# riffusion/riffusion-hobby

Hardware: NVIDIA H100
Metric: clips/sec (higher is better)
Workload: dtype f16

## Files before the change

### riffusion-hobby_b200/csrc/rf_gemm.cu

```cuda
#include <cuda.h>
#include <cuda_fp16.h>
#include <cuda_runtime.h>

#include <algorithm>
#include <cstdio>
#include <cstdlib>
#include <mutex>
#include <string>
#include <vector>

#include "rf_common.h"
#include "rf_tc.cuh"

namespace {

constexpr int BM = 128;
constexpr int BK = 64;
constexpr int A_TILE_BYTES = BM * BK * 2;
constexpr int GEMM_THREADS = 256 + 32;
constexpr int STAGE_PAD = 4;

__host__ __device__ constexpr int stage_bytes(int BN) { return BM * (BN + STAGE_PAD) * 4; }

struct TcParams {
    int M, N, K;
    int batch1, batch2;
    int num_kb;
    int tiles_m, tiles_n;
    int a_m1, a_m2, b_m1, b_m2;
    int conv;
    int taps;
    int kc1, kc2;
    int stride, pad;
    int tap_w;
    int off_x, off_y;
    int osx, osy, oox, ooy;
    int HoF, WoF;
    int Ho, Wo, Bn;
    int bw, bh, bb;
    int tiles_x, tiles_y;
    __half* out;
    long ldo, so1, so2;
    const __half* bias;
    int bias_mode;
    const __half* bias2;
    int bias2_pitch;
    const __half* residual;
    long ldr, sr1, sr2;
    float alpha;
    int act;
    float* out_f32;
    int splits, kb_per_split;
    float* ws;
    long ws_split_stride;
};

__device__ __forceinline__ float apply_act(float v, int act) {
    if (act == 1) return __fdividef(v, 1.f + __expf(-v));
    if (act == 3) return __fdividef(v, 1.f + __expf(-1.702f * v));
    return v;
}

__device__ __forceinline__ float gelu_erf_fast(float g) {
    const float t = fminf(fabsf(g) * 0.70710678118654752f, 4.0f);
    float q = -2.1777638e-05f;
    q = fmaf(q, t, 0.0005068331f);
    q = fmaf(q, t, -0.005339398f);
    q = fmaf(q, t, 0.034231447f);
    q = fmaf(q, t, -0.15289085f);
    q = fmaf(q, t, -0.91675895f);
    q = fmaf(q, t, -1.6281544f);
    q = fmaf(q, t, -0.9999938f);
    float h;
    asm("ex2.approx.ftz.f32 %0, %1;" : "=f"(h) : "f"(q));
    return g * (g < 0.f ? (t < 4.0f ? h : 0.f) : 1.f - h);
}

__device__ __forceinline__ void named_bar_sync(int id, int n) { asm volatile("bar.sync %0, %1;" ::"r"(id), "r"(n) : "memory"); }

constexpr int BRES_KB = 5;
template <int BN, int STAGES, bool BRES = false>
__global__ void __launch_bounds__(GEMM_THREADS, 1)
k_tc_gemm(const __grid_constant__ CUtensorMap mapA0, const __grid_constant__ CUtensorMap mapA1,
          const __grid_constant__ CUtensorMap mapB, const TcParams p) {
    extern __shared__ __align__(1024) uint8_t smem[];
    rf_pdl_trigger();
    constexpr int B_TILE_BYTES = BN * BK * 2;
    constexpr int PITCH = BN + STAGE_PAD;
    uint8_t* sA = smem;
    uint8_t* sB = smem + STAGES * A_TILE_BYTES;
    float* stg = reinterpret_cast<float*>(sB + (BRES ? BRES_KB : STAGES) * B_TILE_BYTES);
    uint64_t* full = reinterpret_cast<uint64_t*>(reinterpret_cast<uint8_t*>(stg) + stage_bytes(BN));
    uint64_t* empty = full + STAGES;
    uint64_t* b_full = empty + STAGES;

    const int warp = threadIdx.x >> 5, lane = threadIdx.x & 31;
    const int tiles_mn = p.tiles_n * p.tiles_m;
    const int n_tiles = tiles_mn * p.batch1 * p.batch2 * p.splits;
    const int nb_fixed = BRES ? static_cast<int>(blockIdx.x) % p.tiles_n : 0;
    const int unit0 = BRES ? static_cast<int>(blockIdx.x) / p.tiles_n : blockIdx.x;
    const int unit_step = BRES ? static_cast<int>(gridDim.x) / p.tiles_n : gridDim.x;
    const int n_units = BRES ? p.tiles_m : n_tiles;

    if (threadIdx.x == 0) {
        for (int i = 0; i < STAGES; ++i) {
            tc::mbar_init(&full[i], 1);
            tc::mbar_init(&empty[i], 256);
        }
        tc::mbar_init(b_full, 1);
        tc::fence_barrier_init();
    }
    if (warp == 8 && lane == 0) {
        tc::tma_prefetch_desc(&mapA0);
        tc::tma_prefetch_desc(&mapB);
    }
    __syncthreads();
    rf_pdl_wait();

    if (warp == 8) {
        if (lane != 0) return;
        int it = 0;
        if constexpr (BRES) {
            tc::mbar_expect_tx(b_full, p.num_kb * B_TILE_BYTES);
            for (int kb = 0; kb < p.num_kb; ++kb)
                tc::tma_load_4d(&mapB, b_full, sB + kb * B_TILE_BYTES, kb * BK, nb_fixed * BN, 0, 0);
        }
        for (int unit = unit0; unit < n_units; unit += unit_step) {
            const int tile = BRES ? unit * p.tiles_n + nb_fixed : unit / p.splits, sp = BRES ? 0 : unit - (unit / p.splits) * p.splits;
            const int kb0 = sp * p.kb_per_split, kb1 = min(p.num_kb, kb0 + p.kb_per_split);
            const int z = tile / tiles_mn, mn = tile - z * tiles_mn;
            const int m_blk = mn / p.tiles_n, n_blk = mn - m_blk * p.tiles_n;
            const int b1 = z % p.batch1, b2 = z / p.batch1;
            int tx = 0, ty = 0, tb = 0;
            if (p.conv) {
                tx = m_blk % p.tiles_x;
                ty = (m_blk / p.tiles_x) % p.tiles_y;
                tb = m_blk / (p.tiles_x * p.tiles_y);
            }
            for (int kb = kb0; kb < kb1; ++kb, ++it) {
                const int stage = it % STAGES;
                const uint32_t phase = (it / STAGES) & 1;
                tc::mbar_wait(&empty[stage], phase ^ 1);
                tc::mbar_expect_tx(&full[stage], A_TILE_BYTES + (BRES ? 0 : B_TILE_BYTES));
                void* dstA = sA + stage * A_TILE_BYTES;
                void* dstB = sB + stage * B_TILE_BYTES;
                if (!p.conv) {
                    tc::tma_load_4d(&mapA0, &full[stage], dstA, kb * BK, m_blk * BM, b1 * p.a_m1, b2 * p.a_m2);
                    if (!BRES) tc::tma_load_4d(&mapB, &full[stage], dstB, kb * BK, n_blk * BN, b1 * p.b_m1, b2 * p.b_m2);
                } else {
                    const int kct = p.kc1 + p.kc2;
                    const int tap = kb / kct, kc = kb - tap * kct;
                    const int dy = tap / p.tap_w, dx = tap - dy * p.tap_w;
                    const int x0 = tx * p.bw * p.stride + dx - p.pad + p.off_x;
                    const int y0 = ty * p.bh * p.stride + dy - p.pad + p.off_y;
                    if (kc < p.kc1)
                        tc::tma_load_4d(&mapA0, &full[stage], dstA, kc * BK, x0, y0, tb * p.bb);
                    else
                        tc::tma_load_4d(&mapA1, &full[stage], dstA, (kc - p.kc1) * BK, x0, y0, tb * p.bb);
                    if (!BRES) tc::tma_load_4d(&mapB, &full[stage], dstB, kb * BK, n_blk * BN, 0, 0);
                }
            }
        }
        return;
    }

    const int wg = warp >> 2;
    const int frag_row = wg * 64 + (warp & 3) * 16 + (lane >> 2), frag_col = 2 * (lane & 3);
    const int row = threadIdx.x & 127;
    const int half_id = threadIdx.x >> 7;
    auto ld64 = [](const __half* src, uint4* q4) {
        const uint4* s4 = reinterpret_cast<const uint4*>(src);
#pragma unroll
        for (int j = 0; j < 4; ++j) q4[j] = s4[j];
    };
    if constexpr (BRES) tc::mbar_wait(b_full, 0);
    int it = 0;
    for (int unit = unit0; unit < n_units; unit += unit_step) {
        const int tile = BRES ? unit * p.tiles_n + nb_fixed : unit / p.splits, sp = BRES ? 0 : unit - (unit / p.splits) * p.splits;
        const int kb0 = sp * p.kb_per_split, kb1 = min(p.num_kb, kb0 + p.kb_per_split);
        float acc[BN / 2];
#pragma unroll
        for (int i = 0; i < BN / 2; ++i) acc[i] = 0.f;
        int prev = -1;
        for (int kb = kb0; kb < kb1; ++kb, ++it) {
            const int stage = it % STAGES;
            tc::mbar_wait(&full[stage], (it / STAGES) & 1);
            const uint32_t a_base = tc::smem_u32(sA + stage * A_TILE_BYTES) + wg * (64 * 128);
            const uint32_t b_base = tc::smem_u32(sB + (BRES ? kb : stage) * B_TILE_BYTES);
            tc::wgmma_fence();
#pragma unroll
            for (int k = 0; k < BK / 16; ++k)
                tc::wgmma_ss<BN>(acc, tc::make_desc_sw128(a_base + k * 32), tc::make_desc_sw128(b_base + k * 32), 1u);
            tc::wgmma_commit();
            tc::wgmma_wait<1>();
            tc::reg_fence<BN / 2>(acc);
            if (prev >= 0) tc::mbar_arrive(&empty[prev]);
            prev = stage;
        }
        tc::wgmma_wait<0>();
        tc::reg_fence<BN / 2>(acc);
        if (prev >= 0) tc::mbar_arrive(&empty[prev]);

        named_bar_sync(1, 256);
#pragma unroll
        for (int i = 0; i < BN / 8; ++i) {
            const int c = 8 * i + frag_col;
            *reinterpret_cast<float2*>(stg + frag_row * PITCH + c) = make_float2(acc[4 * i], acc[4 * i + 1]);
            *reinterpret_cast<float2*>(stg + (frag_row + 8) * PITCH + c) = make_float2(acc[4 * i + 2], acc[4 * i + 3]);
        }
        named_bar_sync(1, 256);

        const int z = tile / tiles_mn, mn = tile - z * tiles_mn;
        const int m_blk = mn / p.tiles_n, n_blk = mn - m_blk * p.tiles_n;
        const int b1 = z % p.batch1, b2 = z / p.batch1;
        bool row_ok;
        long out_off, res_off;
        int img = 0;
        if (!p.conv) {
            const int m = m_blk * BM + row;
            row_ok = m < p.M;
            out_off = static_cast<long>(b2) * p.so2 + static_cast<long>(b1) * p.so1 + static_cast<long>(m) * p.ldo;
            res_off = static_cast<long>(b2) * p.sr2 + static_cast<long>(b1) * p.sr1 + static_cast<long>(m) * p.ldr;
        } else {
            const int tx = m_blk % p.tiles_x, ty = (m_blk / p.tiles_x) % p.tiles_y, tb = m_blk / (p.tiles_x * p.tiles_y);
            const int xi = row % p.bw, yi = (row / p.bw) % p.bh, bi = row / (p.bw * p.bh);
            const int x = tx * p.bw + xi, y = ty * p.bh + yi;
            img = tb * p.bb + bi;
            row_ok = (x < p.Wo) && (y < p.Ho) && (img < p.Bn);
            const long pix = (static_cast<long>(img) * p.HoF + (y * p.osy + p.ooy)) * p.WoF + (x * p.osx + p.oox);
            out_off = pix * p.ldo;
            res_off = pix * p.ldr;
        }
        const int m_glob = m_blk * BM + row;
        const float bias_row = (p.bias_mode == 2 && row_ok) ? __half2float(p.bias[m_glob]) : 0.f;
#pragma unroll 1
        for (int c0 = half_id * 32; c0 < BN; c0 += 64) {
            const int n0 = n_blk * BN + c0;
            if (!row_ok || n0 >= p.N) continue;
            float f[32];
#pragma unroll
            for (int i = 0; i < 8; ++i) {
                const float4 t = *reinterpret_cast<const float4*>(stg + row * PITCH + c0 + 4 * i);
                f[4 * i] = t.x; f[4 * i + 1] = t.y; f[4 * i + 2] = t.z; f[4 * i + 3] = t.w;
            }
            if (p.splits > 1) {
                float* wp = p.ws + sp * p.ws_split_stride + (out_off / p.ldo) * p.N + n0;
                if (n0 + 32 <= p.N && (p.N & 3) == 0) {
#pragma unroll
                    for (int i = 0; i < 8; ++i)
                        reinterpret_cast<float4*>(wp)[i] = make_float4(f[4 * i], f[4 * i + 1], f[4 * i + 2], f[4 * i + 3]);
                } else {
                    for (int i = 0; i < 32; ++i)
                        if (n0 + i < p.N) wp[i] = f[i];
                }
                continue;
            }
#pragma unroll
            for (int i = 0; i < 32; ++i) f[i] = f[i] * p.alpha + bias_row;
            const bool full_run = n0 + 32 <= p.N;
            if (p.bias_mode == 1) {
                if (full_run && ((reinterpret_cast<uintptr_t>(p.bias + n0) & 15) == 0)) {
                    uint4 q4[4];
                    ld64(p.bias + n0, q4);
#pragma unroll
                    for (int j = 0; j < 4; ++j) {
                        const uint4 bv = q4[j];
                        const __half2* bh = reinterpret_cast<const __half2*>(&bv);
#pragma unroll
                        for (int e = 0; e < 4; ++e) {
                            const float2 t = __half22float2(bh[e]);
                            f[8 * j + 2 * e] += t.x;
                            f[8 * j + 2 * e + 1] += t.y;
                        }
                    }
                } else {
                    for (int i = 0; i < 32; ++i)
                        if (n0 + i < p.N) f[i] += __half2float(p.bias[n0 + i]);
                }
            }
            if (p.bias2) {
                const __half* b2p = p.bias2 + static_cast<long>(img) * p.bias2_pitch + n0;
                if (full_run && ((reinterpret_cast<uintptr_t>(b2p) & 15) == 0)) {
                    uint4 q4[4];
                    ld64(b2p, q4);
#pragma unroll
                    for (int j = 0; j < 4; ++j) {
                        const uint4 bv = q4[j];
                        const __half2* bh = reinterpret_cast<const __half2*>(&bv);
#pragma unroll
                        for (int e = 0; e < 4; ++e) {
                            const float2 t = __half22float2(bh[e]);
                            f[8 * j + 2 * e] += t.x;
                            f[8 * j + 2 * e + 1] += t.y;
                        }
                    }
                } else {
                    for (int i = 0; i < 32; ++i)
                        if (n0 + i < p.N) f[i] += __half2float(b2p[i]);
                }
            }
            if (p.act == 2) {
                __half* dst = p.out + out_off + (n0 >> 1);
                uint32_t pk[8];
#pragma unroll
                for (int j = 0; j < 8; ++j) {
                    const float g0 = f[16 + 2 * j], g1 = f[17 + 2 * j];
                    const float y0 = f[2 * j] * gelu_erf_fast(g0);
                    const float y1 = f[2 * j + 1] * gelu_erf_fast(g1);
                    const __half2 h = __floats2half2_rn(y0, y1);
                    pk[j] = *reinterpret_cast<const uint32_t*>(&h);
                }
                reinterpret_cast<uint4*>(dst)[0] = make_uint4(pk[0], pk[1], pk[2], pk[3]);
                reinterpret_cast<uint4*>(dst)[1] = make_uint4(pk[4], pk[5], pk[6], pk[7]);
                continue;
            }
            if (p.act) {
#pragma unroll
                for (int i = 0; i < 32; ++i) f[i] = apply_act(f[i], p.act);
            }
            if (p.residual) {
                const __half* rp = p.residual + res_off + n0;
                if (full_run && ((reinterpret_cast<uintptr_t>(rp) & 15) == 0)) {
                    uint4 q4[4];
                    ld64(rp, q4);
#pragma unroll
                    for (int j = 0; j < 4; ++j) {
                        const uint4 rv = q4[j];
                        const __half2* rh = reinterpret_cast<const __half2*>(&rv);
#pragma unroll
                        for (int e = 0; e < 4; ++e) {
                            const float2 t = __half22float2(rh[e]);
                            f[8 * j + 2 * e] += t.x;
                            f[8 * j + 2 * e + 1] += t.y;
                        }
                    }
                } else {
                    for (int i = 0; i < 32; ++i)
                        if (n0 + i < p.N) f[i] += __half2float(rp[i]);
                }
            }
            if (p.out_f32) {
                for (int i = 0; i < 32; ++i)
                    if (n0 + i < p.N) p.out_f32[out_off + n0 + i] = f[i];
            } else if (full_run && ((reinterpret_cast<uintptr_t>(p.out + out_off + n0) & 15) == 0)) {
                uint4* dst = reinterpret_cast<uint4*>(p.out + out_off + n0);
#pragma unroll
                for (int i = 0; i < 4; ++i) {
                    __half2 h0 = __floats2half2_rn(f[8 * i + 0], f[8 * i + 1]);
                    __half2 h1 = __floats2half2_rn(f[8 * i + 2], f[8 * i + 3]);
                    __half2 h2 = __floats2half2_rn(f[8 * i + 4], f[8 * i + 5]);
                    __half2 h3 = __floats2half2_rn(f[8 * i + 6], f[8 * i + 7]);
                    dst[i] = make_uint4(*reinterpret_cast<uint32_t*>(&h0), *reinterpret_cast<uint32_t*>(&h1),
                                        *reinterpret_cast<uint32_t*>(&h2), *reinterpret_cast<uint32_t*>(&h3));
                }
            } else {
                for (int i = 0; i < 32; ++i)
                    if (n0 + i < p.N) p.out[out_off + n0 + i] = __float2half_rn(f[i]);
            }
        }
    }
}

struct TcProfile {
    bool on = false;
    std::vector<cudaEvent_t> ev;
    double flops = 0.0;
    long launches = 0;
    struct Rec { int conv, M, N, K, batch, splits, bn; };
    std::vector<Rec> recs;
};

TcProfile g_prof;
std::mutex g_prof_mu;

template <int BN, int STAGES, bool BRES = false>
int launch(const CUtensorMap& a0, const CUtensorMap& a1, const CUtensorMap& b, const TcParams& p, dim3 grid,
           cudaStream_t st) {
    constexpr size_t smem = static_cast<size_t>(STAGES) * A_TILE_BYTES +
                            static_cast<size_t>(BRES ? BRES_KB : STAGES) * (BN * BK * 2) + stage_bytes(BN) + 1024;
    static_assert(smem <= 232448, "shared memory budget (227 KB per block)");
    const int num_sms = rf_num_sms();
    const int n_tiles = static_cast<int>(grid.x * grid.y * grid.z);
    if (BRES) {
        grid = dim3(static_cast<unsigned>((num_sms / p.tiles_n) * p.tiles_n));
    } else {
        grid = dim3(static_cast<unsigned>(n_tiles < num_sms ? n_tiles : num_sms));
    }
    static rf_dev_once once;
    const cudaError_t aerr = rf_set_smem_once(once, k_tc_gemm<BN, STAGES, BRES>, int(smem));
    if (aerr != cudaSuccess) return rf_fail(RF_ERR_CUDA, std::string("cudaFuncSetAttribute: ") + cudaGetErrorString(aerr));
    cudaEvent_t e0 = nullptr, e1 = nullptr;
    const bool prof = g_prof.on;
    if (prof) {
        RF_CUDA_TRY(cudaEventCreate(&e0));
        RF_CUDA_TRY(cudaEventCreate(&e1));
        RF_CUDA_TRY(cudaEventRecord(e0, st));
    }
    RF_LAUNCH_PDL("k_tc_gemm", (k_tc_gemm<BN, STAGES, BRES>), grid, dim3(GEMM_THREADS), smem, st, n_tiles <= 2 * num_sms,
                  a0, a1, b, p);
    if (prof) {
        RF_CUDA_TRY(cudaEventRecord(e1, st));
        std::lock_guard<std::mutex> lk(g_prof_mu);
        g_prof.ev.push_back(e0);
        g_prof.ev.push_back(e1);
        g_prof.launches += 1;
        const double m = p.conv ? static_cast<double>(p.Bn) * p.Ho * p.Wo : static_cast<double>(p.M) * p.batch1 * p.batch2;
        g_prof.flops += 2.0 * m * p.N * p.K;
        g_prof.recs.push_back({p.conv, p.conv ? p.Bn * p.Ho * p.Wo : p.M, p.N, p.K, p.batch1 * p.batch2, p.splits,
                               BRES ? 1000 + BN : BN});
    }
    return RF_OK;
}

__global__ void k_splitk_reduce(const float* __restrict__ ws, int splits, long split_stride, long rows, int N, long ldo,
                                long ldr, int rows_per_image, float alpha, const __half* __restrict__ bias, int bias_mode,
                                const __half* __restrict__ bias2, int bias2_pitch, int act,
                                const __half* __restrict__ residual, __half* __restrict__ out, float* __restrict__ out_f32) {
    const int n8 = N / 8;
    for (long i = static_cast<long>(blockIdx.x) * blockDim.x + threadIdx.x; i < rows * n8;
         i += static_cast<long>(gridDim.x) * blockDim.x) {
        const long r = i / n8;
        const int n0 = static_cast<int>(i - r * n8) * 8;
        float f[8];
#pragma unroll
        for (int e = 0; e < 8; ++e) f[e] = 0.f;
        for (int sidx = 0; sidx < splits; ++sidx) {
            const float4* wp = reinterpret_cast<const float4*>(ws + sidx * split_stride + r * N + n0);
            const float4 a = wp[0], b = wp[1];
            f[0] += a.x; f[1] += a.y; f[2] += a.z; f[3] += a.w;
            f[4] += b.x; f[5] += b.y; f[6] += b.z; f[7] += b.w;
        }
        const float brow = bias_mode == 2 ? __half2float(bias[r]) : 0.f;
#pragma unroll
        for (int e = 0; e < 8; ++e) {
            float v = f[e] * alpha + brow;
            if (bias_mode == 1) v += __half2float(bias[n0 + e]);
            if (bias2) v += __half2float(bias2[(r / rows_per_image) * bias2_pitch + n0 + e]);
            if (act == 1 || act == 3) v = apply_act(v, act);
            if (residual) v += __half2float(residual[r * ldr + n0 + e]);
            f[e] = v;
        }
        if (out_f32) {
#pragma unroll
            for (int e = 0; e < 8; ++e) out_f32[r * ldo + n0 + e] = f[e];
        } else {
            uint32_t pk[4];
#pragma unroll
            for (int e = 0; e < 4; ++e) {
                const __half2 h = __floats2half2_rn(f[2 * e], f[2 * e + 1]);
                pk[e] = *reinterpret_cast<const uint32_t*>(&h);
            }
            *reinterpret_cast<uint4*>(out + r * ldo + n0) = make_uint4(pk[0], pk[1], pk[2], pk[3]);
        }
    }
}

constexpr size_t SPLIT_WS_MAX = static_cast<size_t>(192) << 20;

int pick_splits(long rows, int N, int tiles, int num_kb, int num_sms, bool allowed) {
    static const char* env = getenv("RF_GEMM_SPLITK");
    if (!allowed || (env && env[0] == '0')) return 1;
    const double t_slab = 0.2, t_launch = 3.0, ws_bw = 8.0e6;
    int best = 1;
    double best_t = 1e30;
    for (int S = 1; S <= 8; ++S) {
        if (S > 1 && (num_kb / S < 6 || static_cast<size_t>(S) * rows * N * 4 > SPLIT_WS_MAX)) break;
        const int kbs = (num_kb + S - 1) / S;
        if (S > 1 && (S - 1) * kbs >= num_kb) continue;
        const int waves = (tiles * S + num_sms - 1) / num_sms;
        double t = waves * kbs * t_slab;
        if (S > 1) t += t_launch + 2.0 * S * rows * N * 4 / ws_bw;
        if (env && atoi(env) == S) return S;
        if (t < best_t * (S > 1 ? 0.9 : 1.0)) {
            best_t = t;
            best = S;
        }
    }
    return best;
}

int pick_bn(int N, long tiles_m) {
    if (const char* env = getenv("RF_GEMM_BN")) {
        const int bn = atoi(env);
        if (bn == 64 || bn == 128 || (bn == 160 && N % 160 == 0)) return bn;
    }
    if (N <= 64) return 64;
    if (N % 160) return 128;
    const long sms = rf_num_sms();
    const long t128 = tiles_m * ((N + 127) / 128), t160 = tiles_m * (N / 160);
    const long c128 = ((t128 + sms - 1) / sms) * 128, c160 = ((t160 + sms - 1) / sms) * 160;
    return c160 * 100 <= c128 * 102 ? 160 : 128;
}

int dispatch(int N, int bn, const CUtensorMap& a0, const CUtensorMap& a1, const CUtensorMap& b, TcParams& p,
             int tiles_m, int nbatch, cudaStream_t st, void* ws, size_t ws_bytes, size_t* query) {
    p.tiles_n = (N + bn - 1) / bn;
    p.tiles_m = tiles_m;
    const long rows = p.conv ? static_cast<long>(p.Bn) * p.Ho * p.Wo : p.M;
    const bool can_split = nbatch == 1 && p.act != 2 && (N % 8) == 0 && (p.ldo % 8) == 0 && (!p.conv || p.osx == 1) &&
                           (!p.residual || (p.ldr % 8) == 0) &&
                           ((reinterpret_cast<uintptr_t>(p.out ? static_cast<void*>(p.out) : static_cast<void*>(p.out_f32)) & 15) == 0);
    p.splits = pick_splits(rows, N, p.tiles_n * tiles_m, p.num_kb, rf_num_sms(), can_split);
    p.kb_per_split = (p.num_kb + p.splits - 1) / p.splits;
    p.ws = nullptr;
    p.ws_split_stride = rows * N;
    if (p.splits > 1) {
        const size_t need = static_cast<size_t>(p.splits) * rows * N * sizeof(float);
        if (query) {
            *query = need;
            return RF_OK;
        }
        if (!ws || ws_bytes < need) {
            p.splits = 1;
            p.kb_per_split = p.num_kb;
        } else {
            p.ws = static_cast<float*>(ws);
        }
    }
    if (query) {
        *query = 0;
        return RF_OK;
    }
    dim3 grid(p.tiles_n * p.splits, tiles_m, nbatch);
    int rc;
    const char* env_bres = getenv("RF_GEMM_BRES");
    if (bn == 160 && nbatch == 1 && p.splits == 1 && p.num_kb <= BRES_KB && p.tiles_n <= 8 &&
        static_cast<long>(tiles_m) * p.tiles_n >= 4L * rf_num_sms() && !(env_bres && env_bres[0] == '0')) {
        return launch<160, 2, true>(a0, a1, b, p, grid, st);
    }
    if (bn == 160) rc = launch<160, 3>(a0, a1, b, p, grid, st);
    else if (bn == 128) rc = launch<128, 4>(a0, a1, b, p, grid, st);
    else rc = launch<64, 6>(a0, a1, b, p, grid, st);
    if (rc || p.splits == 1) return rc;
    const long work = rows * (N / 8);
    const unsigned blocks = static_cast<unsigned>(std::min<long>((work + 255) / 256, 8L * rf_num_sms()));
    k_splitk_reduce<<<blocks, 256, 0, st>>>(p.ws, p.splits, p.ws_split_stride, rows, N, p.ldo, p.ldr,
                                            p.conv ? p.Ho * p.Wo : 1, p.alpha, p.bias, p.bias_mode, p.bias2, p.bias2_pitch,
                                            p.act, p.residual, p.out, p.out_f32);
    RF_CUDA_LAUNCH_CHECK("k_splitk_reduce");
    if (g_prof.on) {
        std::lock_guard<std::mutex> lk(g_prof_mu);
        if (!g_prof.ev.empty()) RF_CUDA_TRY(cudaEventRecord(g_prof.ev.back(), st));
    }
    return RF_OK;
}

}

typedef CUresult (*PFN_encodeTiled)(CUtensorMap*, CUtensorMapDataType, cuuint32_t, void*, const cuuint64_t*,
                                    const cuuint64_t*, const cuuint32_t*, const cuuint32_t*, CUtensorMapInterleave,
                                    CUtensorMapSwizzle, CUtensorMapL2promotion, CUtensorMapFloatOOBfill);

static PFN_encodeTiled get_encode() {
    static PFN_encodeTiled fn = nullptr;
    static std::once_flag once;
    std::call_once(once, [] {
        void* sym = nullptr;
        cudaDriverEntryPointQueryResult qres;
        if (cudaGetDriverEntryPoint("cuTensorMapEncodeTiled", &sym, cudaEnableDefault, &qres) == cudaSuccess &&
            qres == cudaDriverEntryPointSuccess)
            fn = reinterpret_cast<PFN_encodeTiled>(sym);
    });
    return fn;
}

int rf_tma_map_f16(CUtensorMap* map, const void* ptr, const long dims[4], const long strides[4], const int box[4],
                   const int estrides[4]) {
    PFN_encodeTiled enc = get_encode();
    if (!enc) return rf_fail(RF_ERR_CUDA, "cuTensorMapEncodeTiled unavailable (no CUDA driver)");
    cuuint64_t gdim[4], gstr[3];
    cuuint32_t bx[4], es[4];
    for (int i = 0; i < 4; ++i) {
        gdim[i] = static_cast<cuuint64_t>(dims[i]);
        bx[i] = static_cast<cuuint32_t>(box[i]);
        es[i] = static_cast<cuuint32_t>(estrides[i]);
        if (i) {
            gstr[i - 1] = static_cast<cuuint64_t>(strides[i]) * 2;
            if (gstr[i - 1] % 16) return rf_fail(RF_ERR_INVALID, "tensor map: stride not a multiple of 16 bytes");
        }
    }
    if (reinterpret_cast<uintptr_t>(ptr) % 16) return rf_fail(RF_ERR_INVALID, "tensor map: base not 16-byte aligned");
    CUresult r = enc(map, CU_TENSOR_MAP_DATA_TYPE_FLOAT16, 4, const_cast<void*>(ptr), gdim, gstr, bx, es,
                     CU_TENSOR_MAP_INTERLEAVE_NONE, CU_TENSOR_MAP_SWIZZLE_128B, CU_TENSOR_MAP_L2_PROMOTION_L2_256B,
                     CU_TENSOR_MAP_FLOAT_OOB_FILL_NONE);
    if (r != CUDA_SUCCESS) return rf_fail(RF_ERR_CUDA, "cuTensorMapEncodeTiled failed: " + std::to_string(int(r)));
    return RF_OK;
}

static int gemm_impl(const rf_gemm_desc* d, void* stream, size_t* query) {
    if (!d || !d->A || !d->B || !d->D || d->M <= 0 || d->N <= 0 || d->K <= 0)
        return rf_fail(RF_ERR_INVALID, "rf_gemm_f16: bad argument");
    const int b1 = d->batch1 > 0 ? d->batch1 : 1, b2 = d->batch2 > 0 ? d->batch2 : 1;
    const int a_m1 = (b1 > 1 && d->sa1 != 0) ? 1 : 0, a_m2 = (b2 > 1 && d->sa2 != 0) ? 1 : 0;
    const int b_m1 = (b1 > 1 && d->sb1 != 0) ? 1 : 0, b_m2 = (b2 > 1 && d->sb2 != 0) ? 1 : 0;
    CUtensorMap ma, mb;
    {
        const long dims[4] = {d->K, d->M, a_m1 ? b1 : 1, a_m2 ? b2 : 1};
        const long str[4] = {1, d->lda, a_m1 ? d->sa1 : d->lda, a_m2 ? d->sa2 : d->lda};
        const int box[4] = {BK, BM, 1, 1};
        const int es[4] = {1, 1, 1, 1};
        int rc = rf_tma_map_f16(&ma, d->A, dims, str, box, es);
        if (rc) return rc;
    }
    const int bn = pick_bn(d->N, static_cast<long>((d->M + BM - 1) / BM) * b1 * b2);
    {
        const long dims[4] = {d->K, d->N, b_m1 ? b1 : 1, b_m2 ? b2 : 1};
        const long str[4] = {1, d->ldb, b_m1 ? d->sb1 : d->ldb, b_m2 ? d->sb2 : d->ldb};
        const int box[4] = {BK, bn, 1, 1};
        const int es[4] = {1, 1, 1, 1};
        int rc = rf_tma_map_f16(&mb, d->B, dims, str, box, es);
        if (rc) return rc;
    }
    TcParams p{};
    p.M = d->M; p.N = d->N; p.K = d->K;
    p.batch1 = b1; p.batch2 = b2;
    p.num_kb = (d->K + BK - 1) / BK;
    p.conv = 0;
    p.a_m1 = a_m1; p.a_m2 = a_m2; p.b_m1 = b_m1; p.b_m2 = b_m2;
    p.out = static_cast<__half*>(d->out_f32 ? nullptr : d->D);
    p.out_f32 = static_cast<float*>(d->out_f32 ? d->D : nullptr);
    p.ldo = d->ldd; p.so1 = d->sd1; p.so2 = d->sd2;
    p.bias = static_cast<const __half*>(d->bias);
    p.bias_mode = d->bias ? d->bias_mode : 0;
    p.bias2 = nullptr;
    p.residual = static_cast<const __half*>(d->residual);
    p.ldr = d->ldr; p.sr1 = d->sr1; p.sr2 = d->sr2;
    p.alpha = d->alpha == 0.f ? 1.f : d->alpha;
    p.act = d->act;
    if (d->act == 2 && ((d->N % 32) || d->residual || d->out_f32 || (d->ldd % 8) || (d->sd1 % 8) || (d->sd2 % 8) ||
                        (reinterpret_cast<uintptr_t>(d->D) & 15)))
        return rf_fail(RF_ERR_UNSUPPORTED, "rf_gemm_f16: GEGLU epilogue needs N % 32 == 0, fp16 output with 16-byte "
                                           "aligned rows and no residual");
    return dispatch(d->N, bn, ma, ma, mb, p, (d->M + BM - 1) / BM, b1 * b2, static_cast<cudaStream_t>(stream), d->workspace,
                    d->workspace_bytes > 0 ? static_cast<size_t>(d->workspace_bytes) : 0, query);
}

extern "C" int rf_gemm_f16(const rf_gemm_desc* d, void* stream) { return gemm_impl(d, stream, nullptr); }
extern "C" size_t rf_gemm_workspace_bytes(const rf_gemm_desc* d) {
    size_t need = 0;
    return gemm_impl(d, nullptr, &need) == RF_OK ? need : 0;
}

static int conv_impl(const rf_conv_desc* d, void* stream, size_t* query) {
    if (!d || !d->x1 || !d->w || !d->out || d->B <= 0 || d->H <= 0 || d->W <= 0 || d->C1 <= 0 || d->Cout <= 0)
        return rf_fail(RF_ERR_INVALID, "rf_conv2d_f16: bad argument");
    const bool up2 = d->pad_mode == 2;
    if (up2 && (d->ksize != 2 || d->stride != 1 || d->x2 || d->residual))
        return rf_fail(RF_ERR_UNSUPPORTED, "rf_conv2d_f16: pad_mode 2 (fused upsample) takes ksize 2 phase weights, stride 1, "
                                           "one input, no residual");
    if (!up2 && d->ksize != 1 && d->ksize != 3) return rf_fail(RF_ERR_UNSUPPORTED, "rf_conv2d_f16: kernel size must be 1 or 3");
    if (d->stride != 1 && d->stride != 2) return rf_fail(RF_ERR_UNSUPPORTED, "rf_conv2d_f16: stride must be 1 or 2");
    if ((d->C1 % BK) || (d->x2 && (d->C2 % BK)))
        return rf_fail(RF_ERR_UNSUPPORTED, "rf_conv2d_f16: channel counts must be multiples of 64 (use the direct "
                                           "convolution for the 4- and 3-channel layers)");
    const int pad = (d->ksize == 3 && d->pad_mode == 0) ? 1 : 0;
    const int extra = (d->ksize == 3 && d->pad_mode == 1) ? 1 : 0;
    const int Ho = up2 ? d->H : (d->H + 2 * pad + extra - d->ksize) / d->stride + 1;
    const int Wo = up2 ? d->W : (d->W + 2 * pad + extra - d->ksize) / d->stride + 1;
    int bw_max = Wo >= 128 ? 128 : Wo;
    while (BM % bw_max) --bw_max;
    int bw = bw_max;
    for (int c = bw_max / 2; c >= 8; c /= 2)
        if ((Wo + c - 1) / c * c < (Wo + bw - 1) / bw * bw) bw = c;
    int bh = BM / bw;
    if (bh > Ho) bh = Ho;
    while ((BM / bw) % bh) --bh;
    const int bb = BM / (bw * bh);
    const int C2 = d->x2 ? d->C2 : 0;
    CUtensorMap m1, m2, mb;
    const int s = d->stride;
    {
        const long dims[4] = {d->C1, d->W, d->H, d->B};
        const long str[4] = {1, d->C1, static_cast<long>(d->W) * d->C1, static_cast<long>(d->H) * d->W * d->C1};
        const int box[4] = {BK, (bw - 1) * s + 1, (bh - 1) * s + 1, bb};
        const int es[4] = {1, s, s, 1};
        int rc = rf_tma_map_f16(&m1, d->x1, dims, str, box, es);
        if (rc) return rc;
    }
    m2 = m1;
    if (d->x2) {
        const long dims[4] = {C2, d->W, d->H, d->B};
        const long str[4] = {1, C2, static_cast<long>(d->W) * C2, static_cast<long>(d->H) * d->W * C2};
        const int box[4] = {BK, (bw - 1) * s + 1, (bh - 1) * s + 1, bb};
        const int es[4] = {1, s, s, 1};
        int rc = rf_tma_map_f16(&m2, d->x2, dims, str, box, es);
        if (rc) return rc;
    }
    const int taps = d->ksize * d->ksize;
    const long Ktot = static_cast<long>(taps) * (d->C1 + C2);
    const long conv_tiles_m = static_cast<long>((Wo + bw - 1) / bw) * ((Ho + bh - 1) / bh) * ((d->B + bb - 1) / bb);
    const int bn = pick_bn(d->Cout, conv_tiles_m);
    {
        const long dims[4] = {Ktot, d->Cout, 1, 1};
        const long str[4] = {1, Ktot, Ktot * d->Cout, Ktot * d->Cout};
        const int box[4] = {BK, bn, 1, 1};
        const int es[4] = {1, 1, 1, 1};
        int rc = rf_tma_map_f16(&mb, d->w, dims, str, box, es);
        if (rc) return rc;
    }
    TcParams p{};
    p.M = 0; p.N = d->Cout; p.K = static_cast<int>(Ktot);
    p.batch1 = 1; p.batch2 = 1;
    p.conv = 1; p.taps = taps;
    p.kc1 = d->C1 / BK; p.kc2 = C2 / BK;
    p.num_kb = taps * (p.kc1 + p.kc2);
    p.stride = s; p.pad = pad;
    p.tap_w = d->ksize; p.off_x = 0; p.off_y = 0;
    p.osx = 1; p.osy = 1; p.oox = 0; p.ooy = 0;
    p.Ho = Ho; p.Wo = Wo; p.Bn = d->B;
    p.HoF = Ho; p.WoF = Wo;
    p.bw = bw; p.bh = bh; p.bb = bb;
    p.tiles_x = (Wo + bw - 1) / bw;
    p.tiles_y = (Ho + bh - 1) / bh;
    const int tiles_b = (d->B + bb - 1) / bb;
    p.out = static_cast<__half*>(d->out);
    p.out_f32 = nullptr;
    p.ldo = d->Cout; p.ldr = d->Cout;
    p.bias = static_cast<const __half*>(d->bias);
    p.bias_mode = d->bias ? 1 : 0;
    p.bias2 = static_cast<const __half*>(d->bias_per_image);
    p.bias2_pitch = d->bias_per_image_pitch > 0 ? d->bias_per_image_pitch : d->Cout;
    p.residual = static_cast<const __half*>(d->residual);
    p.alpha = d->alpha == 0.f ? 1.f : d->alpha;
    p.act = d->act;
    void* ws = d->workspace;
    const size_t ws_bytes = d->workspace_bytes > 0 ? static_cast<size_t>(d->workspace_bytes) : 0;
    if (!up2) return dispatch(d->Cout, bn, m1, m2, mb, p, p.tiles_x * p.tiles_y * tiles_b, 1, static_cast<cudaStream_t>(stream), ws,
                              ws_bytes, query);
    p.osx = 2; p.osy = 2; p.HoF = 2 * Ho; p.WoF = 2 * Wo;
    for (int ph = 0; ph < 4; ++ph) {
        const int py = ph >> 1, px = ph & 1;
        p.off_y = py - 1; p.off_x = px - 1;
        p.ooy = py; p.oox = px;
        CUtensorMap mph;
        const long dims[4] = {Ktot, d->Cout, 1, 1};
        const long str[4] = {1, Ktot, Ktot * d->Cout, Ktot * d->Cout};
        const int box[4] = {BK, bn, 1, 1};
        const int es[4] = {1, 1, 1, 1};
        int rc = rf_tma_map_f16(&mph, static_cast<const __half*>(d->w) + static_cast<long>(ph) * d->Cout * Ktot, dims, str, box, es);
        if (rc) return rc;
        TcParams q = p;
        rc = dispatch(d->Cout, bn, m1, m2, mph, q, p.tiles_x * p.tiles_y * tiles_b, 1, static_cast<cudaStream_t>(stream), nullptr, 0,
                      query);
        if (rc || query) return rc;
    }
    return RF_OK;
}

extern "C" int rf_conv2d_f16(const rf_conv_desc* d, void* stream) { return conv_impl(d, stream, nullptr); }
extern "C" size_t rf_conv2d_workspace_bytes(const rf_conv_desc* d) {
    size_t need = 0;
    return conv_impl(d, nullptr, &need) == RF_OK ? need : 0;
}

extern "C" int rf_tc_profile_begin(void) {
    std::lock_guard<std::mutex> lk(g_prof_mu);
    g_prof.on = true;
    g_prof.flops = 0.0;
    g_prof.launches = 0;
    g_prof.recs.clear();
    for (cudaEvent_t e : g_prof.ev) cudaEventDestroy(e);
    g_prof.ev.clear();
    return RF_OK;
}
extern "C" int rf_tc_profile_end(double* ms_out, double* flops_out, long* launches_out) {
    std::lock_guard<std::mutex> lk(g_prof_mu);
    g_prof.on = false;
    double ms = 0.0;
    cudaError_t err = cudaDeviceSynchronize();
    FILE* dump = nullptr;
    if (const char* path = getenv("RF_TC_PROFILE_DUMP")) dump = fopen(path, "w");
    if (dump) fprintf(dump, "conv,M,N,K,batch,splits,bn,ms\n");
    for (size_t i = 0; i + 1 < g_prof.ev.size() && err == cudaSuccess; i += 2) {
        float t = 0.f;
        err = cudaEventElapsedTime(&t, g_prof.ev[i], g_prof.ev[i + 1]);
        ms += t;
        if (dump && i / 2 < g_prof.recs.size()) {
            const TcProfile::Rec& r = g_prof.recs[i / 2];
            fprintf(dump, "%d,%d,%d,%d,%d,%d,%d,%.4f\n", r.conv, r.M, r.N, r.K, r.batch, r.splits, r.bn, t);
        }
    }
    if (dump) fclose(dump);
    for (cudaEvent_t e : g_prof.ev) cudaEventDestroy(e);
    g_prof.ev.clear();
    if (ms_out) *ms_out = ms;
    if (flops_out) *flops_out = g_prof.flops;
    if (launches_out) *launches_out = g_prof.launches;
    if (err != cudaSuccess) return rf_fail(RF_ERR_CUDA, std::string("rf_tc_profile_end: ") + cudaGetErrorString(err));
    return RF_OK;
}
```

Measured before the change: 3.871.

## Add persistent ping-pong warpgroup GEMM kernel for long-K problems

Adds a persistent warp-specialized GEMM kernel with one TMA producer warp and two consumer warpgroups that alternate tiles. Ordering barriers let one warpgroup's epilogue overlap the other's MMA mainloop. It is selected when K has at least 90 blocks, there is no split-K, and there are enough tiles to fill the SMs. The per-warpgroup smem epilogue buffers reduce pipeline stages, and the added code paths (conv, geglu, residual) carry correctness risk.

```diff
diff --git a/riffusion-hobby_b200/csrc/rf_gemm.cu b/riffusion-hobby_b200/csrc/rf_gemm.cu
--- a/riffusion-hobby_b200/csrc/rf_gemm.cu
+++ b/riffusion-hobby_b200/csrc/rf_gemm.cu
@@ -361,6 +361,280 @@
     }
 }
 
+
+constexpr int PP_THREADS = 384;
+constexpr int PP_MIN_KB = 90;
+constexpr int EPI_PAD = 8;
+__host__ __device__ constexpr int epi_bytes(int BN) { return 64 * (BN + EPI_PAD) * 2 + 64 * 2 * 8; }
+
+__device__ __forceinline__ void named_bar_arrive(int id, int n) { asm volatile("bar.arrive %0, %1;" ::"r"(id), "r"(n) : "memory"); }
+
+constexpr int WG_BAR = 1, ORDER_BAR = 3;
+
+template <int BN, int STAGES>
+__global__ void __launch_bounds__(PP_THREADS, 1)
+k_tc_gemm_pp(const __grid_constant__ CUtensorMap mapA0, const __grid_constant__ CUtensorMap mapA1,
+          const __grid_constant__ CUtensorMap mapB, const TcParams p) {
+    extern __shared__ __align__(1024) uint8_t smem[];
+    rf_pdl_trigger();
+    constexpr int B_TILE_BYTES = BN * BK * 2;
+    constexpr int EP = BN + EPI_PAD;
+    uint8_t* sA = smem;
+    uint8_t* sB = smem + STAGES * A_TILE_BYTES;
+    uint8_t* sE = sB + STAGES * B_TILE_BYTES;
+    uint64_t* full = reinterpret_cast<uint64_t*>(sE + 2 * epi_bytes(BN));
+    uint64_t* empty = full + STAGES;
+
+    const int warp = threadIdx.x >> 5, lane = threadIdx.x & 31;
+    const int tiles_mn = p.tiles_n * p.tiles_m;
+    const int n_tiles = tiles_mn * p.batch1 * p.batch2;
+
+    if (threadIdx.x == 0) {
+        for (int i = 0; i < STAGES; ++i) {
+            tc::mbar_init(&full[i], 1);
+            tc::mbar_init(&empty[i], 128);
+        }
+        tc::fence_barrier_init();
+    }
+    if (warp == 8 && lane == 0) {
+        tc::tma_prefetch_desc(&mapA0);
+        tc::tma_prefetch_desc(&mapB);
+    }
+    __syncthreads();
+    rf_pdl_wait();
+
+    if (warp >= 8) {
+        asm volatile("setmaxnreg.dec.sync.aligned.u32 40;" ::: "memory");
+        if (warp != 8 || lane != 0) return;
+        int it = 0;
+        for (int tile = blockIdx.x; tile < n_tiles; tile += gridDim.x) {
+            const int z = tile / tiles_mn, mn = tile - z * tiles_mn;
+            const int m_blk = mn / p.tiles_n, n_blk = mn - m_blk * p.tiles_n;
+            const int b1 = z % p.batch1, b2 = z / p.batch1;
+            int tx = 0, ty = 0, tb = 0;
+            if (p.conv) {
+                tx = m_blk % p.tiles_x;
+                ty = (m_blk / p.tiles_x) % p.tiles_y;
+                tb = m_blk / (p.tiles_x * p.tiles_y);
+            }
+            for (int kb = 0; kb < p.num_kb; ++kb, ++it) {
+                const int stage = it % STAGES;
+                const uint32_t phase = (it / STAGES) & 1;
+                tc::mbar_wait(&empty[stage], phase ^ 1);
+                tc::mbar_expect_tx(&full[stage], A_TILE_BYTES + B_TILE_BYTES);
+                void* dstA = sA + stage * A_TILE_BYTES;
+                void* dstB = sB + stage * B_TILE_BYTES;
+                if (!p.conv) {
+                    tc::tma_load_4d(&mapA0, &full[stage], dstA, kb * BK, m_blk * BM, b1 * p.a_m1, b2 * p.a_m2);
+                    tc::tma_load_4d(&mapB, &full[stage], dstB, kb * BK, n_blk * BN, b1 * p.b_m1, b2 * p.b_m2);
+                } else {
+                    const int kct = p.kc1 + p.kc2;
+                    const int tap = kb / kct, kc = kb - tap * kct;
+                    const int dy = tap / p.tap_w, dx = tap - dy * p.tap_w;
+                    const int x0 = tx * p.bw * p.stride + dx - p.pad + p.off_x;
+                    const int y0 = ty * p.bh * p.stride + dy - p.pad + p.off_y;
+                    if (kc < p.kc1)
+                        tc::tma_load_4d(&mapA0, &full[stage], dstA, kc * BK, x0, y0, tb * p.bb);
+                    else
+                        tc::tma_load_4d(&mapA1, &full[stage], dstA, (kc - p.kc1) * BK, x0, y0, tb * p.bb);
+                    tc::tma_load_4d(&mapB, &full[stage], dstB, kb * BK, n_blk * BN, 0, 0);
+                }
+            }
+        }
+        return;
+    }
+
+    asm volatile("setmaxnreg.inc.sync.aligned.u32 232;" ::: "memory");
+    const int wg = warp >> 2;
+    const int t = threadIdx.x & 127;
+    __half* ebuf = reinterpret_cast<__half*>(sE + wg * epi_bytes(BN));
+    long* row_out = reinterpret_cast<long*>(ebuf + 64 * EP);
+    long* row_res = row_out + 64;
+    const int frag_row = (t >> 5) * 16 + (lane >> 2), frag_col = 2 * (lane & 3);
+    const int bar_wg = WG_BAR + wg;
+    int it = 0, local = 0;
+    for (int tile = blockIdx.x; tile < n_tiles; tile += gridDim.x, ++local) {
+        if ((local & 1) != wg) {
+            it += p.num_kb;
+            continue;
+        }
+        if (local > 0) named_bar_sync(ORDER_BAR + wg, 256);
+        float acc[BN];
+#pragma unroll
+        for (int i = 0; i < BN; ++i) acc[i] = 0.f;
+        int prev = -1;
+        for (int kb = 0; kb < p.num_kb; ++kb, ++it) {
+            const int stage = it % STAGES;
+            tc::mbar_wait(&full[stage], (it / STAGES) & 1);
+            const uint32_t a_base = tc::smem_u32(sA + stage * A_TILE_BYTES);
+            const uint32_t b_base = tc::smem_u32(sB + stage * B_TILE_BYTES);
+            tc::wgmma_fence();
+#pragma unroll
+            for (int k = 0; k < BK / 16; ++k) {
+                const uint64_t db = tc::make_desc_sw128(b_base + k * 32);
+                tc::wgmma_ss<BN>(acc, tc::make_desc_sw128(a_base + k * 32), db, 1u);
+                tc::wgmma_ss<BN>(acc + BN / 2, tc::make_desc_sw128(a_base + 64 * 128 + k * 32), db, 1u);
+            }
+            tc::wgmma_commit();
+            tc::wgmma_wait<1>();
+            tc::reg_fence<BN>(acc);
+            if (prev >= 0) tc::mbar_arrive(&empty[prev]);
+            prev = stage;
+        }
+        tc::wgmma_wait<0>();
+        tc::reg_fence<BN>(acc);
+        if (prev >= 0) tc::mbar_arrive(&empty[prev]);
+        if (tile + static_cast<int>(gridDim.x) < n_tiles) named_bar_arrive(ORDER_BAR + (wg ^ 1), 256);
+
+        const int z = tile / tiles_mn, mn = tile - z * tiles_mn;
+        const int m_blk = mn / p.tiles_n, n_blk = mn - m_blk * p.tiles_n;
+        const int b1 = z % p.batch1, b2 = z / p.batch1;
+        const int tb = p.conv ? m_blk / (p.tiles_x * p.tiles_y) : 0;
+        const bool geglu = p.act == 2;
+        const bool via_smem = !p.out_f32;
+        const bool res_in = p.residual != nullptr && !geglu;
+#pragma unroll
+        for (int h = 0; h < 2; ++h) {
+            float* f = acc + h * (BN / 2);
+            named_bar_sync(bar_wg, 128);
+            if (t < 64) {
+                const int row = h * 64 + t;
+                bool row_ok;
+                long out_off, res_off;
+                if (!p.conv) {
+                    const int m = m_blk * BM + row;
+                    row_ok = m < p.M;
+                    out_off = static_cast<long>(b2) * p.so2 + static_cast<long>(b1) * p.so1 + static_cast<long>(m) * p.ldo;
+                    res_off = static_cast<long>(b2) * p.sr2 + static_cast<long>(b1) * p.sr1 + static_cast<long>(m) * p.ldr;
+                } else {
+                    const int tx = m_blk % p.tiles_x, ty = (m_blk / p.tiles_x) % p.tiles_y;
+                    const int xi = row % p.bw, yi = (row / p.bw) % p.bh, bi = row / (p.bw * p.bh);
+                    const int x = tx * p.bw + xi, y = ty * p.bh + yi;
+                    const int img = tb * p.bb + bi;
+                    row_ok = (x < p.Wo) && (y < p.Ho) && (img < p.Bn);
+                    const long pix = (static_cast<long>(img) * p.HoF + (y * p.osy + p.ooy)) * p.WoF + (x * p.osx + p.oox);
+                    out_off = pix * p.ldo;
+                    res_off = pix * p.ldr;
+                }
+                row_out[t] = row_ok ? out_off : -1;
+                row_res[t] = res_off;
+            }
+            named_bar_sync(bar_wg, 128);
+            if (res_in) {
+                constexpr int CH = BN / 8, G = 4;
+#pragma unroll 1
+                for (int q0 = t; q0 < 64 * CH; q0 += 128 * G) {
+                    uint4 v[G];
+#pragma unroll
+                    for (int j = 0; j < G; ++j) {
+                        const int q = q0 + 128 * j, r = (q / CH) & 63, c = q % CH;
+                        const int n = n_blk * BN + 8 * c;
+                        const __half* src = p.residual + row_res[r] + n;
+                        if (q < 64 * CH && row_out[r] >= 0 && n + 8 <= p.N && (reinterpret_cast<uintptr_t>(src) & 15) == 0)
+                            v[j] = *reinterpret_cast<const uint4*>(src);
+                    }
+#pragma unroll
+                    for (int j = 0; j < G; ++j) {
+                        const int q = q0 + 128 * j, r = (q / CH) & 63, c = q % CH;
+                        const int n = n_blk * BN + 8 * c;
+                        if (q >= 64 * CH || row_out[r] < 0 || n >= p.N) continue;
+                        const __half* src = p.residual + row_res[r] + n;
+                        __half* dst = ebuf + r * EP + 8 * c;
+                        if (n + 8 <= p.N && (reinterpret_cast<uintptr_t>(src) & 15) == 0) {
+                            *reinterpret_cast<uint4*>(dst) = v[j];
+                        } else {
+                            for (int e = 0; e < 8; ++e)
+                                if (n + e < p.N) dst[e] = src[e];
+                        }
+                    }
+                }
+                named_bar_sync(bar_wg, 128);
+            }
+            long ro[2];
+            float bias_row[2] = {0.f, 0.f};
+            const __half* b2p[2] = {nullptr, nullptr};
+#pragma unroll
+            for (int rr = 0; rr < 2; ++rr) {
+                const int r = frag_row + 8 * rr;
+                ro[rr] = row_out[r];
+                if (ro[rr] < 0) continue;
+                if (p.bias_mode == 2) bias_row[rr] = __half2float(p.bias[m_blk * BM + h * 64 + r]);
+                if (p.bias2) b2p[rr] = p.bias2 + static_cast<long>(tb * p.bb + (h * 64 + r) / (p.bw * p.bh)) * p.bias2_pitch;
+            }
+#pragma unroll
+            for (int i = 0; i < BN / 8; ++i) {
+                const int c = 8 * i + frag_col;
+                const int n = n_blk * BN + c;
+                float bc[2] = {0.f, 0.f};
+                if (p.bias_mode == 1) {
+                    if (n < p.N) bc[0] = __half2float(p.bias[n]);
+                    if (n + 1 < p.N) bc[1] = __half2float(p.bias[n + 1]);
+                }
+#pragma unroll
+                for (int rr = 0; rr < 2; ++rr) {
+                    const int r = frag_row + 8 * rr;
+#pragma unroll
+                    for (int e = 0; e < 2; ++e) {
+                        float v = f[4 * i + 2 * rr + e] * p.alpha + bias_row[rr];
+                        if (p.bias_mode == 1) v += bc[e];
+                        if (b2p[rr] && n + e < p.N) v += __half2float(b2p[rr][n + e]);
+                        if (!geglu && p.act) v = apply_act(v, p.act);
+                        if (res_in) v += __half2float(ebuf[r * EP + c + e]);
+                        f[4 * i + 2 * rr + e] = v;
+                    }
+                }
+            }
+#pragma unroll
+            for (int rr = 0; rr < 2; ++rr) {
+                const int r = frag_row + 8 * rr;
+                if (geglu) {
+#pragma unroll
+                    for (int i = 0; i < BN / 8; ++i) {
+                        if ((i & 3) >= 2) continue;
+                        const float y0 = f[4 * i + 2 * rr] * gelu_erf_fast(f[4 * (i + 2) + 2 * rr]);
+                        const float y1 = f[4 * i + 2 * rr + 1] * gelu_erf_fast(f[4 * (i + 2) + 2 * rr + 1]);
+                        *reinterpret_cast<__half2*>(ebuf + r * EP + 16 * (i >> 2) + 8 * (i & 3) + frag_col) =
+                            __floats2half2_rn(y0, y1);
+                    }
+                } else if (p.out_f32) {
+                    if (ro[rr] < 0) continue;
+#pragma unroll
+                    for (int i = 0; i < BN / 8; ++i) {
+                        const int n = n_blk * BN + 8 * i + frag_col;
+                        if (n < p.N) p.out_f32[ro[rr] + n] = f[4 * i + 2 * rr];
+                        if (n + 1 < p.N) p.out_f32[ro[rr] + n + 1] = f[4 * i + 2 * rr + 1];
+                    }
+                } else {
+#pragma unroll
+                    for (int i = 0; i < BN / 8; ++i)
+                        *reinterpret_cast<__half2*>(ebuf + r * EP + 8 * i + frag_col) =
+                            __floats2half2_rn(f[4 * i + 2 * rr], f[4 * i + 2 * rr + 1]);
+                }
+            }
+            if (via_smem) {
+                named_bar_sync(bar_wg, 128);
+                const int OC = geglu ? BN / 2 : BN;
+                const int n_out = geglu ? p.N / 2 : p.N;
+                const int CH = OC / 8;
+                for (int q = t; q < 64 * CH; q += 128) {
+                    const int r = q / CH, c = q - r * CH;
+                    const int n = n_blk * OC + 8 * c;
+                    const long ro = row_out[r];
+                    if (ro < 0 || n >= n_out) continue;
+                    __half* dst = p.out + ro + n;
+                    const __half* src = ebuf + r * EP + 8 * c;
+                    if (n + 8 <= n_out && (reinterpret_cast<uintptr_t>(dst) & 15) == 0) {
+                        *reinterpret_cast<uint4*>(dst) = *reinterpret_cast<const uint4*>(src);
+                    } else {
+                        for (int e = 0; e < 8; ++e)
+                            if (n + e < n_out) dst[e] = src[e];
+                    }
+                }
+            }
+        }
+    }
+}
+
 struct TcProfile {
     bool on = false;
     std::vector<cudaEvent_t> ev;
@@ -408,6 +682,40 @@
         g_prof.flops += 2.0 * m * p.N * p.K;
         g_prof.recs.push_back({p.conv, p.conv ? p.Bn * p.Ho * p.Wo : p.M, p.N, p.K, p.batch1 * p.batch2, p.splits,
                                BRES ? 1000 + BN : BN});
+    }
+    return RF_OK;
+}
+
+template <int BN, int STAGES>
+int launch_pp(const CUtensorMap& a0, const CUtensorMap& a1, const CUtensorMap& b, const TcParams& p, dim3 grid,
+              cudaStream_t st) {
+    constexpr size_t smem = static_cast<size_t>(STAGES) * (A_TILE_BYTES + BN * BK * 2) + 2 * epi_bytes(BN) +
+                            2 * STAGES * sizeof(uint64_t);
+    static_assert(smem <= 232448, "shared memory budget (227 KB per block)");
+    const int num_sms = rf_num_sms();
+    const int n_tiles = static_cast<int>(grid.x * grid.y * grid.z);
+    grid = dim3(static_cast<unsigned>(n_tiles < num_sms ? n_tiles : num_sms));
+    static rf_dev_once once;
+    const cudaError_t aerr = rf_set_smem_once(once, k_tc_gemm_pp<BN, STAGES>, int(smem));
+    if (aerr != cudaSuccess) return rf_fail(RF_ERR_CUDA, std::string("cudaFuncSetAttribute: ") + cudaGetErrorString(aerr));
+    cudaEvent_t e0 = nullptr, e1 = nullptr;
+    const bool prof = g_prof.on;
+    if (prof) {
+        RF_CUDA_TRY(cudaEventCreate(&e0));
+        RF_CUDA_TRY(cudaEventCreate(&e1));
+        RF_CUDA_TRY(cudaEventRecord(e0, st));
+    }
+    RF_LAUNCH_PDL("k_tc_gemm_pp", (k_tc_gemm_pp<BN, STAGES>), grid, dim3(PP_THREADS), smem, st, n_tiles <= 2 * num_sms,
+                  a0, a1, b, p);
+    if (prof) {
+        RF_CUDA_TRY(cudaEventRecord(e1, st));
+        std::lock_guard<std::mutex> lk(g_prof_mu);
+        g_prof.ev.push_back(e0);
+        g_prof.ev.push_back(e1);
+        g_prof.launches += 1;
+        const double m = p.conv ? static_cast<double>(p.Bn) * p.Ho * p.Wo : static_cast<double>(p.M) * p.batch1 * p.batch2;
+        g_prof.flops += 2.0 * m * p.N * p.K;
+        g_prof.recs.push_back({p.conv, p.conv ? p.Bn * p.Ho * p.Wo : p.M, p.N, p.K, p.batch1 * p.batch2, p.splits, 2000 + BN});
     }
     return RF_OK;
 }
@@ -528,7 +836,11 @@
         static_cast<long>(tiles_m) * p.tiles_n >= 4L * rf_num_sms() && !(env_bres && env_bres[0] == '0')) {
         return launch<160, 2, true>(a0, a1, b, p, grid, st);
     }
-    if (bn == 160) rc = launch<160, 3>(a0, a1, b, p, grid, st);
+    if (p.num_kb >= PP_MIN_KB && p.splits == 1 && static_cast<long>(p.tiles_n) * tiles_m * nbatch >= 2L * rf_num_sms()) {
+        if (bn == 160) rc = launch_pp<160, 5>(a0, a1, b, p, grid, st);
+        else if (bn == 128) rc = launch_pp<128, 5>(a0, a1, b, p, grid, st);
+        else rc = launch_pp<64, 8>(a0, a1, b, p, grid, st);
+    } else if (bn == 160) rc = launch<160, 3>(a0, a1, b, p, grid, st);
     else if (bn == 128) rc = launch<128, 4>(a0, a1, b, p, grid, st);
     else rc = launch<64, 6>(a0, a1, b, p, grid, st);
     if (rc || p.splits == 1) return rc;
```

Result: faster. 4.107 (median of 6 runs) (+6.1%).
